# jzhangbs/MVSDF

Measured on AMD Instinct MI355X. Metric: traced rays/sec (fwd+bwd, 10 sphere iters, 4 src views), higher is better.
Workload: dtype f32x3

## Files before the change

### include/mvsdf_hip.h

```cpp
#ifndef MVSDF_HIP_H
#define MVSDF_HIP_H
#include <stddef.h>
#include <stdint.h>

#ifdef __cplusplus
extern "C" {
#endif

#define MVSDF_MAX_LAYERS 12

typedef struct {
    int n_layers;
    int K[MVSDF_MAX_LAYERS];
    int N[MVSDF_MAX_LAYERS];
    const float* wp[MVSDF_MAX_LAYERS];
    const float* bias[MVSDF_MAX_LAYERS];
    const float* w[MVSDF_MAX_LAYERS];
    int skip_layer;
    int multires;
    const void* wp16[MVSDF_MAX_LAYERS];
    int trace_dtype;
    unsigned skip_mask;
    const void* wx3[MVSDF_MAX_LAYERS];
} MvsdfNetDesc;
// ... 32 lines not shown
size_t mvsdf_packed_floats(int N, int K);

int mvsdf_fold_pack(const float* v, const float* g, int N, int K, float* w, float* wp, float* wpT, void* stream);
int mvsdf_fold_pack_net(int n_layers, const float* const* v, const float* const* g, const int* N, const int* K, float* const* w,
                        float* const* wp, float* const* wpT, void* stream);
int mvsdf_fold_backward_net(int n_layers, const float* const* v, const float* const* g, const float* const* dW, const float* const* db,
                            const int* N, const int* K, float* const* dv, float* const* dg, float* const* dbias, int accumulate,
                            void* stream);
int mvsdf_fold_backward(const float* v, const float* g, const float* dW, int N, int K, float* dv, float* dg, void* stream);

size_t mvsdf_packed_bf16_bytes(int N, int K, int nsplit);
int mvsdf_pack_bf16w_net(int n_layers, const float* const* w, const int* N, const int* K, float* const* wp_rounded, void* stream);
int mvsdf_pack_bf16s_net(int n_layers, const float* const* w, const int* N, const int* K, void* const* wp16, void* stream);
int mvsdf_pack_bf16x3_net(int n_layers, const float* const* w, const int* N, const int* K, void* const* wp16, void* stream);
int mvsdf_pack_bf16x3t_net(int n_layers, const float* const* w, const int* N, const int* K, void* const* wx3t, void* stream);

int mvsdf_sdf_col0(const MvsdfNetDesc* net, const float* x, int n, float* y, int mt, void* stream);

int mvsdf_camera_rays(const float* uv, const float* pose, const float* intrinsics, int B, int P, float* ray_dirs, float* cam_loc,
                      void* stream);

int mvsdf_sphere_intersection(const float* cam_loc, const float* ray_dirs, int B, int P, float r, float* t, uint8_t* mask, void* stream);

size_t mvsdf_trace_workspace_bytes(int R);
size_t mvsdf_trace_workspace_bytes_n(int R, int n_steps);
int mvsdf_trace(const MvsdfNetDesc* net, const MvsdfTraceParams* tp, const float* cam_loc, const float* ray_dirs,
                const uint8_t* object_mask, int B, int P, int training, const float* intervals, const float* minsdf_steps,
                float* points, uint8_t* mask, float* dists, unsigned long long* counters, void* workspace,
                size_t workspace_bytes, int mt, int mt_samples, void* stream);
int mvsdf_trace_stage(int stage, const MvsdfNetDesc* net, const MvsdfTraceParams* tp, const float* cam_loc, const float* ray_dirs,
                      const uint8_t* object_mask, int B, int P, int training, const float* intervals, const float* minsdf_steps,
                      float* points, uint8_t* mask, float* dists, unsigned long long* counters, void* workspace,
                      size_t workspace_bytes, int mt, int mt_samples, void* stream);

size_t mvsdf_tracegen_state_bytes(int R);
int mvsdf_tracegen_init(const MvsdfTraceParams* tp, const float* cam_loc, const float* ray_dirs, const uint8_t* object_mask, int B, int P,
                        void* state, uint8_t* req, float* pts, unsigned long long* counters, void* stream);
int mvsdf_tracegen_step(const MvsdfTraceParams* tp, const float* cam_loc, const float* ray_dirs, int B, int P, void* state, const float* vals,
                        uint8_t* req, float* pts, unsigned long long* counters, void* stream);
int mvsdf_tracegen_finish(const MvsdfTraceParams* tp, const float* cam_loc, const float* ray_dirs, int B, int P, int training, const void* state,
                          float* points, uint8_t* mask, float* dists, unsigned long long* counters, void* workspace, size_t workspace_bytes,
                          void* stream);
int mvsdf_tracegen_rows(const MvsdfTraceParams* tp, int kind, const float* cam_loc, const float* ray_dirs, int B, int P, const float* zs, int n_list,
                        void* workspace, float* out_pts, void* stream);
int mvsdf_tracegen_reduce(const MvsdfTraceParams* tp, int kind, const float* cam_loc, const float* ray_dirs, int B, int P, int training,
                          const float* intervals, const float* minsdf_steps, const float* sv, float* points, uint8_t* mask, float* dists,
                          unsigned long long* counters, void* workspace, uint8_t* marks, void* stream);
int mvsdf_tracegen_secant(const MvsdfTraceParams* tp, int op, const float* cam_loc, const float* ray_dirs, int B, int P, int n_sec, const float* vals,
                          float* pts_out, float* points, float* dists, unsigned long long* counters, void* workspace, void* stream);

size_t mvsdf_sdf_ctx_floats(const MvsdfNetDesc* net, int M, int Mg);
int mvsdf_sdf_forward(const MvsdfNetDesc* net, const MvsdfNetDesc* netT, const float* x, int M, int Mg, float* y, float* nrm, float* ctx,
                      void* stream);
size_t mvsdf_sdf_bwd_ws_floats(const MvsdfNetDesc* net, int Mb);
int mvsdf_sdf_backward(const MvsdfNetDesc* net, const MvsdfNetDesc* netT, const float* x, int M, int Mg, int row0, int Mb, const float* dy,
                       const float* dn, const float* ctx, float* dW_cat, float* db_cat, float* dx, float* ws, void* stream);

int mvsdf_sdf_backward_pair(const MvsdfNetDesc* net, const MvsdfNetDesc* netT, int M, int Mg, int MbA, const float* dyA, const float* dnA, float* wsA,
                            int row0X, int MbX, const float* dyX, const float* dnX, float* wsX, float* dx, const float* ctx, void* stream);
int mvsdf_sdf_backward_finish(const MvsdfNetDesc* net, const MvsdfNetDesc* netT, int M, int Mg, int Mb, const float* dy, const float* ctx, float* ws,
                              int row0D, int MbD, const float* fbar, float* dW_cat, float* db_cat, void* stream);

size_t mvsdf_render_ctx_floats(const MvsdfNetDesc* net, int N);
size_t mvsdf_render_bwd_ws_floats(const MvsdfNetDesc* net, int N);
int mvsdf_render_forward(const MvsdfNetDesc* net, const float* points, const float* view, const float* normals, const float* feat,
                         int ldfeat, int N, int multires_view, float* rgb, float* ctx, void* stream);
// ... 278 lines not shown
```

### mvsdf_amd/_lib.py

```python
import ctypes as C
import os

_HERE = os.path.dirname(os.path.abspath(__file__))
SO_PATH = os.environ.get('MVSDF_LIB') or os.path.join(_HERE, 'libmvsdf_hip.so')
MAX_LAYERS = 12
_lib = None


class NetDesc(C.Structure):
    _fields_ = [('n_layers', C.c_int), ('K', C.c_int * MAX_LAYERS), ('N', C.c_int * MAX_LAYERS),
                ('wp', C.c_void_p * MAX_LAYERS), ('bias', C.c_void_p * MAX_LAYERS), ('w', C.c_void_p * MAX_LAYERS),
                ('skip_layer', C.c_int), ('multires', C.c_int), ('wp16', C.c_void_p * MAX_LAYERS), ('trace_dtype', C.c_int), ('skip_mask', C.c_uint), ('wx3', C.c_void_p * MAX_LAYERS)]


class TraceParams(C.Structure):
    _fields_ = [('r', C.c_float), ('thr', C.c_float), ('line_search_step', C.c_float), ('line_step_iters', C.c_int),
                ('st_iters', C.c_int), ('n_steps', C.c_int), ('n_secant', C.c_int), ('dist_clip', C.c_float)]


class MvsdfError(RuntimeError):
    pass


def lib():
    global _lib
    if _lib is None:
        if not os.path.exists(SO_PATH):
            raise MvsdfError('libmvsdf_hip.so not found at %s -- run `python -c "import __graft_entry__ as g; g.build()"` '
                             '(hipcc --offload-arch=gfx950); there is no CPU/PyTorch fallback for the hot path' % SO_PATH)
        import torch
        L = C.CDLL(SO_PATH)
        L.mvsdf_last_error.restype = C.c_char_p
        L.mvsdf_packed_floats.restype = C.c_size_t
        L.mvsdf_packed_floats.argtypes = [C.c_int, C.c_int]
        L.mvsdf_trace_workspace_bytes.restype = C.c_size_t
        L.mvsdf_trace_workspace_bytes.argtypes = [C.c_int]
        L.mvsdf_trace_workspace_bytes_n.restype = C.c_size_t
        L.mvsdf_trace_workspace_bytes_n.argtypes = [C.c_int, C.c_int]
        for fn in ('mvsdf_sdf_ctx_floats', 'mvsdf_sdf_bwd_ws_floats', 'mvsdf_render_ctx_floats', 'mvsdf_render_bwd_ws_floats'):
            getattr(L, fn).restype = C.c_size_t
        L.mvsdf_adam_ws_floats.restype = C.c_size_t
        L.mvsdf_packed_bf16_bytes.restype = C.c_size_t
        L.mvsdf_packed_bf16_bytes.argtypes = [C.c_int, C.c_int, C.c_int]
        L.mvsdf_tracegen_state_bytes.restype = C.c_size_t
        L.mvsdf_adam_step.argtypes = [C.c_void_p] * 4 + [C.c_size_t] + [C.c_float, C.c_double, C.c_double, C.c_float] + [C.c_int, C.c_float, C.c_void_p, C.c_void_p, C.c_void_p]
        L.mvsdf_adam_step_scaled.argtypes = [C.c_void_p] * 4 + [C.c_size_t] + [C.c_float, C.c_double, C.c_double, C.c_float] + [C.c_int, C.c_float, C.c_float, C.c_void_p, C.c_void_p, C.c_void_p]
        L.mvsdf_adam_step_fused.argtypes = [C.c_void_p] * 4 + [C.c_size_t] + [C.c_float, C.c_double, C.c_double, C.c_float] + [C.c_int, C.c_float, C.c_float, C.c_int, C.c_void_p, C.c_void_p, C.c_void_p]
        L.mvsdf_loss_scale.argtypes = [C.c_void_p] + [C.c_float] * 5 + [C.c_void_p, C.c_void_p, C.c_int] * 4 + [C.c_void_p, C.c_void_p]
        i64, vp, f32 = C.c_int64, C.c_void_p, C.c_float
        L.mvsdf_mc_workspace_bytes.restype = C.c_size_t
        L.mvsdf_mc_workspace_bytes.argtypes = [i64] * 3
        L.mvsdf_mc_count.argtypes = [vp, vp, vp, f32, vp, C.c_size_t, vp]
        L.mvsdf_mc_emit.argtypes = [vp, vp, vp, f32, vp, vp, vp, C.c_size_t, vp, vp, vp, i64, i64, vp]
        L.mvsdf_mesh_cc_workspace_bytes.restype = C.c_size_t
        L.mvsdf_mesh_cc_workspace_bytes.argtypes = [i64, i64]
        L.mvsdf_mesh_components.argtypes = [vp, vp, i64, i64, vp, C.c_size_t, vp, vp, vp]
        L.mvsdf_mesh_select.argtypes = [vp, vp, i64, i64, C.c_int32] + [vp] * 5 + [C.c_size_t] + [vp] * 4 + [i64, i64, vp]
        L.mvsdf_smc_workspace_bytes.restype = C.c_size_t
        L.mvsdf_smc_workspace_bytes.argtypes = [i64, i64]
        L.mvsdf_smc_emit_workspace_bytes.restype = C.c_size_t
        L.mvsdf_smc_emit_workspace_bytes.argtypes = [i64, i64, i64]
        L.mvsdf_smc_coarse_points.argtypes = [vp, i64, i64, i64, i64, vp, vp]
        L.mvsdf_smc_seed.argtypes = [vp, i64, i64, f32, f32, vp, C.c_size_t, vp]
        L.mvsdf_smc_brick_points.argtypes = [vp, i64, i64, vp, C.c_size_t, i64, i64, vp, vp]
        L.mvsdf_smc_closure.argtypes = [vp, i64, i64, f32, i64, i64, vp, C.c_size_t, vp]
        L.mvsdf_smc_count.argtypes = [vp, i64, i64, f32, i64, vp, C.c_size_t, vp, C.c_size_t, vp]
        L.mvsdf_smc_emit.argtypes = [vp, i64, i64, f32, vp, vp, i64, vp, C.c_size_t, vp, C.c_size_t, vp, vp, vp, i64, i64, vp]
        L.mvsdf_mesh_cut_workspace_bytes.restype = C.c_size_t
        L.mvsdf_mesh_cut_workspace_bytes.argtypes = [i64, i64]
        L.mvsdf_mesh_cut.argtypes = [vp, vp, i64, i64, C.c_int32, C.c_int32, vp, C.c_size_t, vp, vp]
        L.mvsdf_mesh_trim.argtypes = [vp] * 4 + [i64, i64, vp, C.c_size_t] + [vp] * 4 + [i64, i64, vp]
# ... 33 lines not shown
        L.mvsdf_featext_raw_floats.argtypes = []
        L.mvsdf_featext_pack_bytes.argtypes = []
        L.mvsdf_featext_pack.argtypes = [vp, vp, sz, vp]
        L.mvsdf_featext_workspace_bytes.argtypes = [i64] * 3
        L.mvsdf_featext_forward.argtypes = [vp, vp, i64, i64, i64, vp, sz, vp, vp, vp, C.c_int, C.c_int, vp]
        L.mvsdf_featext_layer_workspace_bytes.argtypes = [C.c_int] * 5
        L.mvsdf_featext_layer.argtypes = [C.c_int, vp, vp, C.c_int, C.c_int, C.c_int, vp, C.c_int, vp, C.c_int, i64, i64, i64, vp, C.c_int, vp, sz, vp, vp]
        for fn in ('mvsdf_stereo_workspace_bytes', 'mvsdf_stereo_volume_offset'):
            getattr(L, fn).restype = sz
            getattr(L, fn).argtypes = [i64] * 4
        L.mvsdf_stereo_normalize.argtypes = [vp, i64, i64, vp, vp, vp]
        L.mvsdf_stereo_patches.argtypes = [vp, i64, i64, i64, i32, vp, vp]
        L.mvsdf_stereo_sweep.argtypes = [vp, i64, i64, i64, i64, i64] + [vp] * 7 + [sz] + [vp] * 5
        L.mvsdf_viewsel_bits_bytes.restype = sz
        L.mvsdf_viewsel_bits_bytes.argtypes = [i64, i64]
        L.mvsdf_viewsel_workspace_bytes.restype = sz
        L.mvsdf_viewsel_workspace_bytes.argtypes = [i64]
        L.mvsdf_viewsel_pack_dense.argtypes = [vp, i64, i64, vp, vp, vp]
        L.mvsdf_viewsel_pack_tracks.argtypes = [vp, vp, i64, i64, i64, vp, vp, vp]
        L.mvsdf_viewsel_scores.argtypes = [vp, vp, vp, i64, i64, f64, f64, f64, vp, sz, vp, vp, vp, vp]
        L.mvsdf_viewsel_depths.argtypes = [vp, vp, vp, i64, i64, i64, i64, vp, vp, vp]
        L.mvsdf_viewsel_weights_host.argtypes = [vp, vp, i64, f64, f64, f64, vp, vp]
        L.mvsdf_batch_args_bytes.restype = sz
        L.mvsdf_batch_args_bytes.argtypes = []
        L.mvsdf_batch_gather.argtypes = [vp, vp]
        for name in EXPORTS:
            getattr(L, name)
        _lib = L
    return _lib


EXPORTS = [
    'mvsdf_version', 'mvsdf_abi_struct_sizes', 'mvsdf_last_error', 'mvsdf_packed_floats', 'mvsdf_fold_pack', 'mvsdf_fold_backward', 'mvsdf_fold_pack_net', 'mvsdf_fold_backward_net', 'mvsdf_packed_bf16_bytes', 'mvsdf_pack_bf16w_net', 'mvsdf_pack_bf16s_net', 'mvsdf_pack_bf16x3_net', 'mvsdf_pack_bf16x3t_net',
    'mvsdf_sdf_col0', 'mvsdf_camera_rays', 'mvsdf_sphere_intersection', 'mvsdf_trace_workspace_bytes', 'mvsdf_trace_workspace_bytes_n', 'mvsdf_trace', 'mvsdf_trace_stage', 'mvsdf_det_math',
    'mvsdf_tracegen_state_bytes', 'mvsdf_tracegen_init', 'mvsdf_tracegen_step', 'mvsdf_tracegen_finish', 'mvsdf_tracegen_rows', 'mvsdf_tracegen_reduce',
    'mvsdf_tracegen_secant',
    'mvsdf_sdf_ctx_floats', 'mvsdf_sdf_forward', 'mvsdf_sdf_bwd_ws_floats', 'mvsdf_sdf_backward', 'mvsdf_sdf_backward_pair', 'mvsdf_sdf_backward_finish',
    'mvsdf_feat_corr', 'mvsdf_depth_carve', 'mvsdf_loss_terms', 'mvsdf_loss_prep', 'mvsdf_loss_scale', 'mvsdf_adam_ws_floats', 'mvsdf_adam_step', 'mvsdf_adam_step_scaled', 'mvsdf_adam_step_fused',
    'mvsdf_partition_rays', 'mvsdf_step_outputs', 'mvsdf_step_backward_inputs', 'mvsdf_step_backward_fbar', 'mvsdf_dsurf_select', 'mvsdf_dsurf_points',
    'mvsdf_render_ctx_floats', 'mvsdf_render_bwd_ws_floats', 'mvsdf_render_forward', 'mvsdf_render_backward',
    'mvsdf_step_create', 'mvsdf_step_destroy', 'mvsdf_step_forward', 'mvsdf_step_wait_counts', 'mvsdf_step_backward', 'mvsdf_step_set_timing', 'mvsdf_step_trace_times', 'mvsdf_step_times',
    'mvsdf_step_seq', 'mvsdf_step_counts_offset', 'mvsdf_step_wait_counts_seq', 'mvsdf_step_done_seq', 'mvsdf_step_can_defer', 'mvsdf_step_saved_offsets',
    'mvsdf_loss_layout', 'mvsdf_loss_forward', 'mvsdf_loss_backward',
    'mvsdf_mc_workspace_bytes', 'mvsdf_mc_count', 'mvsdf_mc_emit', 'mvsdf_mesh_cc_workspace_bytes', 'mvsdf_mesh_components', 'mvsdf_mesh_select',
    'mvsdf_smc_workspace_bytes', 'mvsdf_smc_emit_workspace_bytes', 'mvsdf_smc_coarse_points', 'mvsdf_smc_seed', 'mvsdf_smc_brick_points',
    'mvsdf_smc_closure', 'mvsdf_smc_count', 'mvsdf_smc_emit',
    'mvsdf_mesh_cut_workspace_bytes', 'mvsdf_mesh_cut', 'mvsdf_mesh_trim',
    'mvsdf_chamfer_key', 'mvsdf_chamfer_sample_workspace_bytes', 'mvsdf_chamfer_sample_count', 'mvsdf_chamfer_sample_emit',
    'mvsdf_chamfer_downsample_workspace_bytes', 'mvsdf_chamfer_downsample', 'mvsdf_chamfer_mask_workspace_bytes', 'mvsdf_chamfer_mask',
    'mvsdf_chamfer_nearest_workspace_bytes', 'mvsdf_chamfer_nearest',
    'mvsdf_fusion_workspace_bytes', 'mvsdf_fusion_fuse', 'mvsdf_fusion_emit',
    'mvsdf_cloud_clean_workspace_bytes', 'mvsdf_cloud_compact_workspace_bytes', 'mvsdf_cloud_knn', 'mvsdf_cloud_components', 'mvsdf_cloud_clean',
    'mvsdf_cloud_compact',
    'mvsdf_raster_workspace_bytes', 'mvsdf_raster_draw', 'mvsdf_raster_resolve', 'mvsdf_raster_visibility', 'mvsdf_raster_colors',
    'mvsdf_featext_raw_floats', 'mvsdf_featext_pack_bytes', 'mvsdf_featext_pack', 'mvsdf_featext_workspace_bytes', 'mvsdf_featext_forward',
    'mvsdf_featext_layer_workspace_bytes', 'mvsdf_featext_layer',
    'mvsdf_stereo_workspace_bytes', 'mvsdf_stereo_volume_offset', 'mvsdf_stereo_normalize', 'mvsdf_stereo_patches', 'mvsdf_stereo_sweep',
    'mvsdf_viewsel_bits_bytes', 'mvsdf_viewsel_workspace_bytes', 'mvsdf_viewsel_pack_dense', 'mvsdf_viewsel_pack_tracks', 'mvsdf_viewsel_scores',
    'mvsdf_viewsel_depths', 'mvsdf_viewsel_weights_host',
    'mvsdf_batch_args_bytes', 'mvsdf_batch_gather',
]


def check(rc, what=''):
    if rc != 0:
        raise MvsdfError('%s failed (code %d): %s' % (what or 'mvsdf call', rc, lib().mvsdf_last_error().decode()))

# ... 14 lines not shown
```

### mvsdf_amd/csrc/trace.hip

```cpp
#include <stdlib.h>
#include <type_traits>
#include "tile_engine.h"
#include "tile_engine_bf16.h"
#include "tile_engine_bf16s.h"
#include "trace_params.h"
#include "capi_util.h"

struct RayCommon {
    float c[3], d[3];
};

__device__ __forceinline__ float mv_clamp(float v, float lo, float hi) { return v < lo ? lo : (v > hi ? hi : v); }

__device__ __forceinline__ bool mv_sphere_isect(const float* c, const float* d, float r, float& t0, float& t1) {
    const float dot = fmaf(d[2], c[2], fmaf(d[1], c[1], d[0] * c[0]));
    const float nrm = sqrtf(c[0] * c[0] + c[1] * c[1] + c[2] * c[2]);
    const float under = dot * dot - (nrm * nrm - r * r);
    const bool hit = under > 0.0f;
    float a = 0.0f, b = 0.0f;
    if (hit) {
        const float s = sqrtf(under);
        a = s * -1.0f - dot;
        b = s * 1.0f - dot;
    }
// ... 323 lines not shown
                    }
                }
            }
            for (int o = 32; o > 0; o >>= 1) used += __shfl_xor(used, o);
            if (lane == 0) nrows_total += (unsigned long long)used;
        }
    }

    if (tail.enable) {
        if (tid == 0 && h_units) atomicAdd(&counters[MV_CNT_TAIL_ROWS], (unsigned long long)h_units * (unsigned long long)ROWS);
        if (tail.probe && tid == 0) {
            unsigned* pr = tail.probe + 4 * blockIdx.x;
            pr[0] = n_rounds; pr[1] = h_units; pr[2] = (unsigned)(clk1 - clk0); pr[3] = (unsigned)((long long)wall_clock64() - clk1);
        }
    }
}

struct SampleCtx {
    const float* cam_loc; const float* dirs; int R, P, training, RPW;
    const float* intervals; const float* steps;
    float* o_points; uint8_t* o_mask; float* o_dists;
    const float* w_zmin; const float* w_zmax;
    float* sec_state;
    int* sec_list;
    float* sv;
    int* list_rest; int* src_rest;
    int n_first;
    unsigned long long* counters;
};

struct RowSeg { const int* list; const int* src; int cnt_index, i0, ni, blocks; int unit_rows; };

template <int MT, int NTW, int NW, class NET>
__device__ void mv_eval_rows(const NET& net, const MvTraceParams& tp, const SampleCtx& c, const RowSeg& sg, long long q0, float* smem, int n_list) {
    constexpr int ROWS = 16 * MT;
    const int tid = threadIdx.x;
    const int n_steps = tp.n_steps, ni = sg.ni;
    const long long total = (long long)n_list * ni;
    if (q0 >= total) return;
    const int nr = (int)min((long long)ROWS, total - q0);
    TraceLds lds = mv_carve<NET>(smem, ROWS, net.S, 3 + 6 * net.multires, 0);
    long long svi = 0;
    if (tid < ROWS) {
        float* p = lds.pts + tid * 3;
        if (tid < nr) {
            const long long q = q0 + tid;
            const int it = (int)(q / ni), i = sg.i0 + (int)(q - (long long)it * ni);
            const int e = sg.list[it];
            const int gid = e & 0x0fffffff;
            const bool samp = (e >> 28) & MV_ITEM_SAMPLER;
            const float* cc = c.cam_loc + 3 * (gid / c.P);
            const float* d = c.dirs + 3 * (size_t)gid;
            const float zmin = c.w_zmin[gid], zmax = c.w_zmax[gid];
            const float z = samp ? (zmin + c.intervals[i] * (zmax - zmin))
                                 : (c.steps[i] * (zmax - zmin) + zmin);
            p[0] = cc[0] + z * d[0]; p[1] = cc[1] + z * d[1]; p[2] = cc[2] + z * d[2];
            svi = (long long)(sg.src ? sg.src[it] : it) * n_steps + i;
        } else { p[0] = 0.f; p[1] = 0.f; p[2] = 0.f; }
    }
    __syncthreads();
    mv_eval_dispatch<MT, NTW, NW>(net, (nr + 15) >> 4, lds.act, lds.pe, lds.pts, lds.sdfv, tid);
    if (tid < nr) c.sv[svi] = lds.sdfv[tid];
}

__device__ __forceinline__ int mv_first_where(const float* __restrict__ sv, int n, int lane, int what) {
    for (int base = 0; base < n; base += 64) {
        const int i = base + lane;
        const float v = i < n ? sv[i] : 1.0f;
        const unsigned long long m = __ballot(what == 0 ? (v < 0.f) : (!(v > 0.f) && !(v < 0.f)));
        if (m) return base + __builtin_ctzll(m);
    }
    return -1;
}
// ... 79 lines not shown
                }
            }
        } else {
            if (it == 0 && lead) atomicAdd(&c.counters[MV_CNT_ROWS_MINSDF], (unsigned long long)n_list * (unsigned long long)n_steps);
            const int bi = mv_first_argmin(sv, n_steps, lane);
            if (lead) { dist = c.steps[bi] * (zmax - zmin) + zmin; have_dist = true; }
        }
        if (lead && have_dist) {
            c.o_dists[gid] = dist;
            c.o_points[3 * (size_t)gid + 0] = cc[0] + dist * d[0];
            c.o_points[3 * (size_t)gid + 1] = cc[1] + dist * d[1];
            c.o_points[3 * (size_t)gid + 2] = cc[2] + dist * d[2];
        }
    }
    if (mode == 2) return;
    if (lead) s_cat[w] = cat;
    __syncthreads();
    if (threadIdx.x == 0) {
        unsigned n1 = 0, n2 = 0;
        for (int k = 0; k < MV_RED_WAVES; ++k) { n1 += s_cat[k] == 1; n2 += s_cat[k] == 2; }
        if (n1) s_base[0] = atomicAdd(&c.counters[MV_CNT_N_SAMPLER_REST], (unsigned long long)n1);
        if (n2) s_base[1] = atomicAdd(&c.counters[MV_CNT_N_SECANT], (unsigned long long)n2);
    }
    __syncthreads();
    if (lead && cat) {
        unsigned rank = 0;
        for (int k = 0; k < w; ++k) rank += s_cat[k] == cat;
        const unsigned long long k = s_base[cat - 1] + rank;
        if (cat == 1) { c.list_rest[k] = e; c.src_rest[k] = it; }
        else c.sec_list[k] = gid;
    }
}

template <int MT, int NTW, int NW, class NET>
__device__ void mv_secant_rays(const NET& net, const MvTraceParams& tp, const SampleCtx& c, int n_list, int block, float* smem) {
    constexpr int ROWS = 16 * MT;
    const int tid = threadIdx.x;
    const int r0 = block * ROWS;
    if (r0 >= n_list) return;
    const int n = min(ROWS, n_list - r0);
    TraceLds lds = mv_carve<NET>(smem, ROWS, net.S, 3 + 6 * net.multires, 0);
    const bool mine = tid < n;
    int gid = 0;
    float cc[3] = {0, 0, 0}, d[3] = {0, 0, 0}, z_low = 0, z_high = 0, sdf_low = 0, sdf_high = 1, z_pred = 0;
    if (mine) {
        gid = c.sec_list[r0 + tid];
        const int b = gid / c.P;
        for (int i = 0; i < 3; ++i) { cc[i] = c.cam_loc[3 * b + i]; d[i] = c.dirs[3 * (size_t)gid + i]; }
        z_low = c.sec_state[gid]; z_high = c.sec_state[(size_t)c.R + gid];
        sdf_low = c.sec_state[2 * (size_t)c.R + gid]; sdf_high = c.sec_state[3 * (size_t)c.R + gid];
        z_pred = -sdf_low * (z_high - z_low) / (sdf_high - sdf_low) + z_low;
    }
    for (int it = 0; it < tp.n_secant; ++it) {
        if (tid < ROWS) { float* p = lds.pts + tid * 3; p[0] = cc[0] + z_pred * d[0]; p[1] = cc[1] + z_pred * d[1]; p[2] = cc[2] + z_pred * d[2]; }
        __syncthreads();
        mv_eval_dispatch<MT, NTW, NW>(net, (n + 15) >> 4, lds.act, lds.pe, lds.pts, lds.sdfv, tid);
        if (mine) {
            const float sm = lds.sdfv[tid];
            if (sm > 0.f) { z_low = z_pred; sdf_low = sm; }
            if (sm < 0.f) { z_high = z_pred; sdf_high = sm; }
            z_pred = -sdf_low * (z_high - z_low) / (sdf_high - sdf_low) + z_low;
        }
    }
    if (mine) {
        c.o_dists[gid] = z_pred;
        c.o_points[3 * (size_t)gid + 0] = cc[0] + z_pred * d[0];
        c.o_points[3 * (size_t)gid + 1] = cc[1] + z_pred * d[1];
        c.o_points[3 * (size_t)gid + 2] = cc[2] + z_pred * d[2];
    }
    if (tid == 0) atomicAdd(&c.counters[MV_CNT_ROWS_SECANT], (unsigned long long)n * (unsigned long long)tp.n_secant);
}

template <class NET> struct mv_net_wt { static constexpr int v = 1; };
template <int NS, int WT> struct mv_net_wt<MvNetBs<NS, WT>> { static constexpr int v = WT; };
template <int MT, int NTW, int NW, class NET>
__global__ __launch_bounds__(64 * NW, (mv_net_wt<NET>::v == 3 && NTW == 2 && MT <= 2 && NW == 8) ? 4 : NW / 4) void k_ray_samples(NET net, MvTraceParams tp, SampleCtx c, RowSeg s0, RowSeg s1, int sec_blocks) {
    extern __shared__ __attribute__((aligned(16))) float smem[];
    int b = blockIdx.x;
    if (b < sec_blocks) {
        mv_secant_rays<(MT > 1 ? 1 : MT), NTW, NW, NET>(net, tp, c, (int)c.counters[MV_CNT_N_SECANT], b, smem);
        return;
    }
    b -= sec_blocks;
    const bool first = b < s0.blocks;
    if (!first && b - s0.blocks >= s1.blocks) return;
    const RowSeg sg = first ? s0 : s1;
    long long q0 = (long long)(first ? b : b - s0.blocks) * (16 * MT);
    const int n_list = (int)c.counters[sg.cnt_index];
    if (sg.unit_rows > 0) {
        if (q0 >= (long long)n_list * sg.ni + 16 * MT) return;
        __shared__ long long s_q0;
        if (threadIdx.x == 0) s_q0 = (long long)atomicAdd(&c.counters[MV_CNT_TAIL_NEXT], (unsigned long long)(16 * MT));
        __syncthreads();
        q0 = s_q0;
    }
    mv_eval_rows<MT, NTW, NW, NET>(net, tp, c, sg, q0, smem, n_list);
}
static int mv_tail_mode() {
    static int v = -1;
    if (v < 0) { const char* e = getenv("MVSDF_TAIL"); v = e ? atoi(e) : 1; }
    return v;
}
static unsigned* g_tail_probe = nullptr;
static unsigned* mv_tail_probe() { return g_tail_probe; }
extern "C" void mv_trace_set_tail_probe(unsigned* buf) { g_tail_probe = buf; }
static float* mv_minsdf_sv(float* ws, int R, int n_steps) {
    float* sec_state = ws + 2 * (size_t)R;
    int* w_list = (int*)(sec_state + 4 * (size_t)R);
    float* sv = (float*)(w_list + 3 * (size_t)R);
    int* list_rest = (int*)(sv + (size_t)R * n_steps);
    return (float*)(list_rest + 2 * (size_t)R);
}

static int mv_cu_count() {
    static int n = 0;
    if (n == 0) {
        int dev = 0, v = 0;
        if (hipGetDevice(&dev) != hipSuccess || hipDeviceGetAttribute(&v, hipDeviceAttributeMultiprocessorCount, dev) != hipSuccess || v <= 0) { (void)hipGetLastError(); v = 1; }
        n = v;
    }
    return n;
}
template <class NET>
static bool mv_tail_on(int training, const float* steps, int R, int mt1) {
    constexpr bool is_bf = !std::is_same<NET, MvNet>::value;
    const int grid1 = (R + 8 * mt1 - 1) / (8 * mt1);
    const int need = !is_bf ? 1 : ((mv_net_wt<NET>::v == 3 && R > 2048) ? 1 : 2);
    return training && steps && mv_tail_mode() >= need && grid1 <= mv_cu_count();
}

template <class NET>
static size_t trace_lds_bytes(const NET& net, int MT, int sv_floats, int rpw, bool sphere = false) {
    const int rows = 16 * MT, d0 = 3 + 6 * net.multires;
    size_t f = (size_t)mv_act_rows<NET>(rows, sphere) * net.S + ((rows * d0 + 3) & ~3) + rows * 4 + rows + sv_floats;
    return f * 4 + 16 + (size_t)rpw * (8 * 4 + 4) + 16;
}

template <int MT, int NTW, int NW, class NET>
// ... 33 lines not shown

template <int MT, int NTW, int NW, class NET>
static hipError_t launch_stage2(const NET& net, const MvTraceParams& tp, const float* cam_loc, const float* dirs, int B, int P, int training,
                                const float* intervals, const float* steps, float* points, uint8_t* mask, float* dists, float* ws,
                                unsigned long long* counters, int parts, int mt1, hipStream_t stream) {
    const int R = B * P, ROWS = 16 * MT;
    float* w_zmin = ws;
    float* w_zmax = w_zmin + R;
    float* sec_state = w_zmax + R;
    int* w_list = (int*)(sec_state + 4 * (size_t)R);
    int* w_list_min = w_list + R;
    int* sec_list = w_list_min + R;
    float* sv = (float*)(sec_list + R);
    const size_t lds2 = trace_lds_bytes(net, MT, 0, 0);
    static size_t set2 = 0;
    if (lds2 > set2) {
        hipError_t e = hipFuncSetAttribute((const void*)k_ray_samples<MT, NTW, NW, NET>, hipFuncAttributeMaxDynamicSharedMemorySize, (int)lds2);
        if (e != hipSuccess) return e;
        set2 = lds2;
    }
    static int nf_env = -1;
    if (nf_env < 0) { const char* e = mv_dev_env("MVSDF_NFIRST"); nf_env = e ? atoi(e) : 12; if (nf_env < 2) nf_env = 2; }
    const int n = tp.n_steps, nf = nf_env < n ? nf_env : n;
    SampleCtx c;
    c.cam_loc = cam_loc; c.dirs = dirs; c.R = R; c.P = P; c.training = training; c.RPW = 0; c.intervals = intervals; c.steps = steps;
    c.o_points = points; c.o_mask = mask; c.o_dists = dists; c.w_zmin = w_zmin; c.w_zmax = w_zmax; c.sec_state = sec_state;
    c.sec_list = sec_list; c.sv = sv; c.counters = counters;
    c.list_rest = (int*)(sv + (size_t)R * n); c.src_rest = c.list_rest + R; c.n_first = nf;
    auto blocks_for = [&](int per_item) { return (int)(((long long)R * per_item + ROWS - 1) / ROWS); };
    const int sec_blocks = (R + 15) / 16, red_blocks = (R + MV_RED_WAVES - 1) / MV_RED_WAVES;
    const RowSeg none = {nullptr, nullptr, 0, 0, 1, 0, 0};
    if (parts & 1) {
        const RowSeg first = {w_list, nullptr, (int)MV_CNT_N_SAMPLER, 0, nf, blocks_for(nf), 0};
        hipLaunchKernelGGL((k_ray_samples<MT, NTW, NW, NET>), dim3(first.blocks), dim3(64 * NW), lds2, stream, net, tp, c, first, none, 0);
        hipLaunchKernelGGL(k_reduce_items, dim3(red_blocks), dim3(64 * MV_RED_WAVES), 0, stream, tp, c, w_list, (const int*)nullptr, (int)MV_CNT_N_SAMPLER, 0);
        if (nf < n) {
            const RowSeg rest = {c.list_rest, c.src_rest, (int)MV_CNT_N_SAMPLER_REST, nf, n - nf, blocks_for(n - nf), 0};
            hipLaunchKernelGGL((k_ray_samples<MT, NTW, NW, NET>), dim3(rest.blocks), dim3(64 * NW), lds2, stream, net, tp, c, rest, none, 0);
            hipLaunchKernelGGL(k_reduce_items, dim3(red_blocks), dim3(64 * MV_RED_WAVES), 0, stream, tp, c, c.list_rest, c.src_rest, (int)MV_CNT_N_SAMPLER_REST, 1);
        }
    }
    if (parts & 2) {
        const bool tail = mv_tail_on<NET>(training, steps, R, mt1);
        SampleCtx cm = c;
        if (tail) cm.sv = mv_minsdf_sv(ws, R, n);
        const RowSeg minsdf = {w_list_min, nullptr, (int)MV_CNT_N_MINSDF, 0, n, training ? blocks_for(n) + (tail ? 1 : 0) : 0, tail ? 1 : 0};
        hipLaunchKernelGGL((k_ray_samples<MT, NTW, NW, NET>), dim3(sec_blocks + minsdf.blocks), dim3(64 * NW), lds2, stream, net, tp, cm, minsdf, none,
                           sec_blocks);
        if (training) hipLaunchKernelGGL(k_reduce_items, dim3(red_blocks), dim3(64 * MV_RED_WAVES), 0, stream, tp, cm, w_list_min, (const int*)nullptr, (int)MV_CNT_N_MINSDF, 2);
    }
    if ((parts & 4) && training) {
        SampleCtx c2 = c;
        c2.sv = (float*)(c.src_rest + R);
        const bool tail = mv_tail_on<NET>(training, steps, R, mt1);
        const RowSeg minsdf = {w_list_min, nullptr, (int)MV_CNT_N_MINSDF, 0, n, blocks_for(n) + (tail ? 1 : 0), tail ? 1 : 0};
        hipLaunchKernelGGL((k_ray_samples<MT, NTW, NW, NET>), dim3(minsdf.blocks), dim3(64 * NW), lds2, stream, net, tp, c2, minsdf, none, 0);
        hipLaunchKernelGGL(k_reduce_items, dim3(red_blocks), dim3(64 * MV_RED_WAVES), 0, stream, tp, c2, w_list_min, (const int*)nullptr, (int)MV_CNT_N_MINSDF, 2);
    }
    if (parts & 8)
        hipLaunchKernelGGL((k_ray_samples<MT, NTW, NW, NET>), dim3(sec_blocks), dim3(64 * NW), lds2, stream, net, tp, c, none, none, sec_blocks);
    return hipGetLastError();
}

#ifndef MV_SPHERE_NW16
#define MV_SPHERE_NW16 1
#endif
template <class NET>
hipError_t mv_trace_launch(int stages, const NET& net, const MvTraceParams& tp, int mt1, int mt2, const float* cam_loc, const float* dirs,
                           const uint8_t* om, int B, int P, int training, const float* intervals, const float* steps, float* points,
                           uint8_t* mask, float* dists, float* ws, unsigned long long* counters, hipStream_t stream) {
    int maxnt = 0;
    for (int l = 0; l < net.n_layers - 1; ++l) maxnt = net.L[l].NT > maxnt ? net.L[l].NT : maxnt;
    if (maxnt > 32) return hipErrorInvalidValue;
    constexpr bool is_bf = !std::is_same<NET, MvNet>::value;
    const bool eight = is_bf || maxnt >= 16;
    const bool wide = maxnt > 16;
    hipError_t e = hipSuccess;
    auto eff = [&](int mt) { return wide ? (mt >= 2 ? 2 : 1) : (mt >= 4 ? 4 : (mt >= 2 ? 2 : 1)); };
    const int mt1_eff = eff(mt1), mt2_eff = eff(mt2);
#define MV_S1(MT_, NTW_, NW_) e = launch_stage1<MT_, NTW_, NW_>(net, tp, cam_loc, dirs, om, B, P, training, steps, mt2_eff, points, mask, dists, ws, counters, stream)
#define MV_S2(MT_, NTW_, NW_) e = launch_stage2<MT_, NTW_, NW_>(net, tp, cam_loc, dirs, B, P, training, intervals, steps, points, mask, dists, ws, counters, (stages >> 1) & 15, mt1_eff, stream)
    if (stages & 1) {
        if (eight) {
            if (wide) { if (mt1 >= 2) MV_S1(2, 4, 8); else MV_S1(1, 4, 8); }
            else if (mt1 >= 4) MV_S1(4, 2, 8); else if (mt1 >= 2) MV_S1(2, 2, 8);
            else {
                if constexpr (MV_SPHERE_NW16 != 0 && mv_net_wt<NET>::v == 3) MV_S1(1, 1, 16); else MV_S1(1, 2, 8);
            }
        } else if constexpr (!is_bf) {
            if (wide) { if (mt1 >= 2) MV_S1(2, 8, 4); else MV_S1(1, 8, 4); }
            else if (mt1 >= 4) MV_S1(4, 4, 4); else if (mt1 >= 2) MV_S1(2, 4, 4); else MV_S1(1, 4, 4);
        }
        if (e != hipSuccess) return e;
// ... 276 lines not shown
    if (td == 3)
        e = mv_trace_launch(stages, net2, *tp, mt, rpw, cam_loc, ray_dirs, object_mask, B, P, training, intervals,
                            minsdf_steps ? minsdf_steps : intervals, points, mask, dists, (float*)workspace, counters, s);
    else if (td == 4)
        e = mv_trace_launch(stages, net3, *tp, mt, rpw, cam_loc, ray_dirs, object_mask, B, P, training, intervals,
                            minsdf_steps ? minsdf_steps : intervals, points, mask, dists, (float*)workspace, counters, s);
    else if (td == 5)
        e = mv_trace_launch(stages, net33, *tp, mt, rpw, cam_loc, ray_dirs, object_mask, B, P, training, intervals,
                            minsdf_steps ? minsdf_steps : intervals, points, mask, dists, (float*)workspace, counters, s);
    else
        e = mv_trace_launch(stages, net, *tp, mt, rpw, cam_loc, ray_dirs, object_mask, B, P, training, intervals,
                            minsdf_steps ? minsdf_steps : intervals, points, mask, dists, (float*)workspace, counters, s);
    return mv_check(e, "mvsdf_trace");
}

int mvsdf_trace(const MvsdfNetDesc* desc, const MvsdfTraceParams* tp, const float* cam_loc, const float* ray_dirs,
                const uint8_t* object_mask, int B, int P, int training, const float* intervals, const float* minsdf_steps,
                float* points, uint8_t* mask, float* dists, unsigned long long* counters, void* workspace,
                size_t workspace_bytes, int mt, int rpw, void* stream) {
    return trace_impl(7, desc, tp, cam_loc, ray_dirs, object_mask, B, P, training, intervals, minsdf_steps, points, mask, dists, counters,
                      workspace, workspace_bytes, mt, rpw, stream);
}

int mvsdf_trace_stage(int stage, const MvsdfNetDesc* desc, const MvsdfTraceParams* tp, const float* cam_loc, const float* ray_dirs,
                      const uint8_t* object_mask, int B, int P, int training, const float* intervals, const float* minsdf_steps,
                      float* points, uint8_t* mask, float* dists, unsigned long long* counters, void* workspace,
                      size_t workspace_bytes, int mt, int rpw, void* stream) {
    if (stage < 1 || stage > 6) return mv_fail(-1, "mvsdf_trace_stage: stage must be 1..6");
    static const int bits[7] = {0, 1, 6, 2, 4, 8, 16};
    return trace_impl(bits[stage], desc, tp, cam_loc, ray_dirs, object_mask, B, P, training, intervals, minsdf_steps, points, mask, dists, counters,
                      workspace, workspace_bytes, mt, rpw, stream);
}

int mv_trace_stage1_prezeroed(const MvsdfNetDesc* desc, const MvsdfTraceParams* tp, const float* cam_loc, const float* ray_dirs, const uint8_t* object_mask,
                              int B, int P, int training, const float* intervals, const float* minsdf_steps, float* points, uint8_t* mask, float* dists,
                              unsigned long long* counters, void* workspace, size_t workspace_bytes, int mt, int rpw, void* stream) {
    return trace_impl(1 | 0x100, desc, tp, cam_loc, ray_dirs, object_mask, B, P, training, intervals, minsdf_steps, points, mask, dists, counters,
                      workspace, workspace_bytes, mt, rpw, stream);
}

size_t mvsdf_tracegen_state_bytes(int R) { return (size_t)(R > 0 ? R : 0) * sizeof(GenRay); }

static int tracegen_check(const MvsdfTraceParams* tp, int B, int P) {
    if (!tp || B <= 0 || P <= 0 || (long long)B * P >= (1 << 28)) return mv_fail(-1, "mvsdf_tracegen: bad sizes");
    if (tp->n_steps < 2 || tp->n_steps > 1024 || tp->line_step_iters < 0 || tp->line_step_iters > 30) return mv_fail(-1, "mvsdf_tracegen: tracer parameters out of range");
    return 0;
}

int mvsdf_tracegen_init(const MvsdfTraceParams* tp, const float* cam_loc, const float* ray_dirs, const uint8_t* object_mask, int B, int P,
                        void* state, uint8_t* req, float* pts, unsigned long long* counters, void* stream) {
    int rc = tracegen_check(tp, B, P);
    if (rc) return rc;
    if (!cam_loc || !ray_dirs || !object_mask || !state || !req || !pts || !counters) return mv_fail(-1, "mvsdf_tracegen_init: null argument");
    const int R = B * P;
    hipStream_t s = (hipStream_t)stream;
    hipError_t e = hipMemsetAsync(counters, 0, 16 * sizeof(unsigned long long), s);
    if (e != hipSuccess) return mv_check(e, "mvsdf_tracegen_init: memset");
    hipLaunchKernelGGL(k_gen_init, dim3((R + 255) / 256), dim3(256), 0, s, *tp, cam_loc, ray_dirs, object_mask, R, P, (GenRay*)state, req, pts);
    return mv_check(hipGetLastError(), "mvsdf_tracegen_init");
}

int mvsdf_tracegen_step(const MvsdfTraceParams* tp, const float* cam_loc, const float* ray_dirs, int B, int P, void* state, const float* vals,
                        uint8_t* req, float* pts, unsigned long long* counters, void* stream) {
    int rc = tracegen_check(tp, B, P);
    if (rc) return rc;
    if (!cam_loc || !ray_dirs || !state || !vals || !req || !pts || !counters) return mv_fail(-1, "mvsdf_tracegen_step: null argument");
// ... 78 lines not shown
```

Measured before the change: 1.388 million.

## Balance minsdf row tiles across CUs and let secant use cross-row eval

```diff
diff --git a/include/mvsdf_hip.h b/include/mvsdf_hip.h
--- a/include/mvsdf_hip.h
+++ b/include/mvsdf_hip.h
@@ -88,6 +88,8 @@
                       const uint8_t* object_mask, int B, int P, int training, const float* intervals, const float* minsdf_steps,
                       float* points, uint8_t* mask, float* dists, unsigned long long* counters, void* workspace,
                       size_t workspace_bytes, int mt, int mt_samples, void* stream);
+int mvsdf_trace_row_schedule(long long n_rows, int cus, long long grid_blocks, long long block, int mt_samples, long long* q0, int* nr);
+int mvsdf_trace_set_row_cus(int cus);
 
 size_t mvsdf_tracegen_state_bytes(int R);
 int mvsdf_tracegen_init(const MvsdfTraceParams* tp, const float* cam_loc, const float* ray_dirs, const uint8_t* object_mask, int B, int P,
diff --git a/mvsdf_amd/_lib.py b/mvsdf_amd/_lib.py
--- a/mvsdf_amd/_lib.py
+++ b/mvsdf_amd/_lib.py
@@ -37,6 +37,8 @@
         L.mvsdf_trace_workspace_bytes.argtypes = [C.c_int]
         L.mvsdf_trace_workspace_bytes_n.restype = C.c_size_t
         L.mvsdf_trace_workspace_bytes_n.argtypes = [C.c_int, C.c_int]
+        L.mvsdf_trace_row_schedule.argtypes = [C.c_longlong, C.c_int, C.c_longlong, C.c_longlong, C.c_int, C.POINTER(C.c_longlong), C.POINTER(C.c_int)]
+        L.mvsdf_trace_set_row_cus.argtypes = [C.c_int]
         for fn in ('mvsdf_sdf_ctx_floats', 'mvsdf_sdf_bwd_ws_floats', 'mvsdf_render_ctx_floats', 'mvsdf_render_bwd_ws_floats'):
             getattr(L, fn).restype = C.c_size_t
         L.mvsdf_adam_ws_floats.restype = C.c_size_t
@@ -136,7 +138,7 @@
 
 EXPORTS = [
     'mvsdf_version', 'mvsdf_abi_struct_sizes', 'mvsdf_last_error', 'mvsdf_packed_floats', 'mvsdf_fold_pack', 'mvsdf_fold_backward', 'mvsdf_fold_pack_net', 'mvsdf_fold_backward_net', 'mvsdf_packed_bf16_bytes', 'mvsdf_pack_bf16w_net', 'mvsdf_pack_bf16s_net', 'mvsdf_pack_bf16x3_net', 'mvsdf_pack_bf16x3t_net',
-    'mvsdf_sdf_col0', 'mvsdf_camera_rays', 'mvsdf_sphere_intersection', 'mvsdf_trace_workspace_bytes', 'mvsdf_trace_workspace_bytes_n', 'mvsdf_trace', 'mvsdf_trace_stage', 'mvsdf_det_math',
+    'mvsdf_sdf_col0', 'mvsdf_camera_rays', 'mvsdf_sphere_intersection', 'mvsdf_trace_workspace_bytes', 'mvsdf_trace_workspace_bytes_n', 'mvsdf_trace', 'mvsdf_trace_stage', 'mvsdf_trace_row_schedule', 'mvsdf_trace_set_row_cus', 'mvsdf_det_math',
     'mvsdf_tracegen_state_bytes', 'mvsdf_tracegen_init', 'mvsdf_tracegen_step', 'mvsdf_tracegen_finish', 'mvsdf_tracegen_rows', 'mvsdf_tracegen_reduce',
     'mvsdf_tracegen_secant',
     'mvsdf_sdf_ctx_floats', 'mvsdf_sdf_forward', 'mvsdf_sdf_bwd_ws_floats', 'mvsdf_sdf_backward', 'mvsdf_sdf_backward_pair', 'mvsdf_sdf_backward_finish',
diff --git a/mvsdf_amd/csrc/trace.hip b/mvsdf_amd/csrc/trace.hip
--- a/mvsdf_amd/csrc/trace.hip
+++ b/mvsdf_amd/csrc/trace.hip
@@ -379,13 +379,13 @@
 struct RowSeg { const int* list; const int* src; int cnt_index, i0, ni, blocks; int unit_rows; };
 
 template <int MT, int NTW, int NW, class NET>
-__device__ void mv_eval_rows(const NET& net, const MvTraceParams& tp, const SampleCtx& c, const RowSeg& sg, long long q0, float* smem, int n_list) {
+__device__ void mv_eval_rows(const NET& net, const MvTraceParams& tp, const SampleCtx& c, const RowSeg& sg, long long q0, int lim, float* smem, int n_list) {
     constexpr int ROWS = 16 * MT;
     const int tid = threadIdx.x;
     const int n_steps = tp.n_steps, ni = sg.ni;
     const long long total = (long long)n_list * ni;
     if (q0 >= total) return;
-    const int nr = (int)min((long long)ROWS, total - q0);
+    const int nr = (int)min((long long)lim, total - q0);
     TraceLds lds = mv_carve<NET>(smem, ROWS, net.S, 3 + 6 * net.multires, 0);
     long long svi = 0;
     if (tid < ROWS) {
@@ -531,7 +531,7 @@
     }
 }
 
-template <int MT, int NTW, int NW, class NET>
+template <int MT, int NTW, int NW, class NET, bool XR = false>
 __device__ void mv_secant_rays(const NET& net, const MvTraceParams& tp, const SampleCtx& c, int n_list, int block, float* smem) {
     constexpr int ROWS = 16 * MT;
     const int tid = threadIdx.x;
@@ -553,7 +553,7 @@
     for (int it = 0; it < tp.n_secant; ++it) {
         if (tid < ROWS) { float* p = lds.pts + tid * 3; p[0] = cc[0] + z_pred * d[0]; p[1] = cc[1] + z_pred * d[1]; p[2] = cc[2] + z_pred * d[2]; }
         __syncthreads();
-        mv_eval_dispatch<MT, NTW, NW>(net, (n + 15) >> 4, lds.act, lds.pe, lds.pts, lds.sdfv, tid);
+        mv_eval_dispatch<MT, NTW, NW, NET, (XR && MT == 1)>(net, (n + 15) >> 4, lds.act, lds.pe, lds.pts, lds.sdfv, tid);
         if (mine) {
             const float sm = lds.sdfv[tid];
             if (sm > 0.f) { z_low = z_pred; sdf_low = sm; }
@@ -572,12 +572,31 @@
 
 template <class NET> struct mv_net_wt { static constexpr int v = 1; };
 template <int NS, int WT> struct mv_net_wt<MvNetBs<NS, WT>> { static constexpr int v = WT; };
+
+#ifndef MV_ROWS_BALANCED
+#define MV_ROWS_BALANCED 1
+#endif
+#ifndef MV_SECANT_CARRY
+#define MV_SECANT_CARRY 1
+#endif
+__host__ __device__ inline void mv_row_schedule(long long n_rows, long long C, long long grid, long long b, int rows, long long* q0, int* nr) {
+    const long long nfull = (n_rows / (rows * C)) * C;
+    if (b < nfull) { *q0 = b * rows; *nr = rows; return; }
+    const long long base = nfull * rows, rem = n_rows - base;
+    *q0 = n_rows; *nr = 0;
+    if (rem <= 0) return;
+    long long u = 16 * ((rem + 16 * C - 1) / (16 * C));
+    while (u < rows && nfull + (rem + u - 1) / u > grid) u += 16;
+    const long long s = base + (b - nfull) * u;
+    if (s < n_rows) { *q0 = s; *nr = (int)(n_rows - s < u ? n_rows - s : u); }
+}
+
 template <int MT, int NTW, int NW, class NET>
-__global__ __launch_bounds__(64 * NW, (mv_net_wt<NET>::v == 3 && NTW == 2 && MT <= 2 && NW == 8) ? 4 : NW / 4) void k_ray_samples(NET net, MvTraceParams tp, SampleCtx c, RowSeg s0, RowSeg s1, int sec_blocks) {
+__global__ __launch_bounds__(64 * NW, (mv_net_wt<NET>::v == 3 && NTW == 2 && MT <= 2 && NW == 8) ? 4 : NW / 4) void k_ray_samples(NET net, MvTraceParams tp, SampleCtx c, RowSeg s0, RowSeg s1, int sec_blocks, int row_cus) {
     extern __shared__ __attribute__((aligned(16))) float smem[];
     int b = blockIdx.x;
     if (b < sec_blocks) {
-        mv_secant_rays<(MT > 1 ? 1 : MT), NTW, NW, NET>(net, tp, c, (int)c.counters[MV_CNT_N_SECANT], b, smem);
+        mv_secant_rays<(MT > 1 ? 1 : MT), NTW, NW, NET, (MV_SECANT_CARRY != 0 && MT >= 4 && NW == 8)>(net, tp, c, (int)c.counters[MV_CNT_N_SECANT], b, smem);
         return;
     }
     b -= sec_blocks;
@@ -593,7 +612,15 @@
         __syncthreads();
         q0 = s_q0;
     }
-    mv_eval_rows<MT, NTW, NW, NET>(net, tp, c, sg, q0, smem, n_list);
+    int lim = 16 * MT;
+    constexpr bool HELD128 = mv_net_wt<NET>::v == 3 && NTW == 2 && MT <= 2 && NW == 8;
+    if (MV_ROWS_BALANCED != 0 && !HELD128 && row_cus != 0 && first && sg.unit_rows == 0) {
+        const long long sec_active = ((long long)c.counters[MV_CNT_N_SECANT] + 15) >> 4;
+        const long long C = row_cus < 0 ? -(long long)row_cus : (row_cus - sec_active > 1 ? row_cus - sec_active : 1);
+        mv_row_schedule((long long)n_list * sg.ni, C, s0.blocks, b, 16 * MT, &q0, &lim);
+        if (lim == 0) return;
+    }
+    mv_eval_rows<MT, NTW, NW, NET>(net, tp, c, sg, q0, lim, smem, n_list);
 }
 static int mv_tail_mode() {
     static int v = -1;
@@ -603,6 +630,7 @@
 static unsigned* g_tail_probe = nullptr;
 static unsigned* mv_tail_probe() { return g_tail_probe; }
 extern "C" void mv_trace_set_tail_probe(unsigned* buf) { g_tail_probe = buf; }
+static int g_row_cus = 0;
 static float* mv_minsdf_sv(float* ws, int R, int n_steps) {
     float* sec_state = ws + 2 * (size_t)R;
     int* w_list = (int*)(sec_state + 4 * (size_t)R);
@@ -702,11 +730,11 @@
     const RowSeg none = {nullptr, nullptr, 0, 0, 1, 0, 0};
     if (parts & 1) {
         const RowSeg first = {w_list, nullptr, (int)MV_CNT_N_SAMPLER, 0, nf, blocks_for(nf), 0};
-        hipLaunchKernelGGL((k_ray_samples<MT, NTW, NW, NET>), dim3(first.blocks), dim3(64 * NW), lds2, stream, net, tp, c, first, none, 0);
+        hipLaunchKernelGGL((k_ray_samples<MT, NTW, NW, NET>), dim3(first.blocks), dim3(64 * NW), lds2, stream, net, tp, c, first, none, 0, 0);
         hipLaunchKernelGGL(k_reduce_items, dim3(red_blocks), dim3(64 * MV_RED_WAVES), 0, stream, tp, c, w_list, (const int*)nullptr, (int)MV_CNT_N_SAMPLER, 0);
         if (nf < n) {
             const RowSeg rest = {c.list_rest, c.src_rest, (int)MV_CNT_N_SAMPLER_REST, nf, n - nf, blocks_for(n - nf), 0};
-            hipLaunchKernelGGL((k_ray_samples<MT, NTW, NW, NET>), dim3(rest.blocks), dim3(64 * NW), lds2, stream, net, tp, c, rest, none, 0);
+            hipLaunchKernelGGL((k_ray_samples<MT, NTW, NW, NET>), dim3(rest.blocks), dim3(64 * NW), lds2, stream, net, tp, c, rest, none, 0, 0);
             hipLaunchKernelGGL(k_reduce_items, dim3(red_blocks), dim3(64 * MV_RED_WAVES), 0, stream, tp, c, c.list_rest, c.src_rest, (int)MV_CNT_N_SAMPLER_REST, 1);
         }
     }
@@ -716,7 +744,7 @@
         if (tail) cm.sv = mv_minsdf_sv(ws, R, n);
         const RowSeg minsdf = {w_list_min, nullptr, (int)MV_CNT_N_MINSDF, 0, n, training ? blocks_for(n) + (tail ? 1 : 0) : 0, tail ? 1 : 0};
         hipLaunchKernelGGL((k_ray_samples<MT, NTW, NW, NET>), dim3(sec_blocks + minsdf.blocks), dim3(64 * NW), lds2, stream, net, tp, cm, minsdf, none,
-                           sec_blocks);
+                           sec_blocks, (!training || tail) ? 0 : (g_row_cus > 0 ? -g_row_cus : mv_cu_count()));
         if (training) hipLaunchKernelGGL(k_reduce_items, dim3(red_blocks), dim3(64 * MV_RED_WAVES), 0, stream, tp, cm, w_list_min, (const int*)nullptr, (int)MV_CNT_N_MINSDF, 2);
     }
     if ((parts & 4) && training) {
@@ -724,11 +752,11 @@
         c2.sv = (float*)(c.src_rest + R);
         const bool tail = mv_tail_on<NET>(training, steps, R, mt1);
         const RowSeg minsdf = {w_list_min, nullptr, (int)MV_CNT_N_MINSDF, 0, n, blocks_for(n) + (tail ? 1 : 0), tail ? 1 : 0};
-        hipLaunchKernelGGL((k_ray_samples<MT, NTW, NW, NET>), dim3(minsdf.blocks), dim3(64 * NW), lds2, stream, net, tp, c2, minsdf, none, 0);
+        hipLaunchKernelGGL((k_ray_samples<MT, NTW, NW, NET>), dim3(minsdf.blocks), dim3(64 * NW), lds2, stream, net, tp, c2, minsdf, none, 0, 0);
         hipLaunchKernelGGL(k_reduce_items, dim3(red_blocks), dim3(64 * MV_RED_WAVES), 0, stream, tp, c2, w_list_min, (const int*)nullptr, (int)MV_CNT_N_MINSDF, 2);
     }
     if (parts & 8)
-        hipLaunchKernelGGL((k_ray_samples<MT, NTW, NW, NET>), dim3(sec_blocks), dim3(64 * NW), lds2, stream, net, tp, c, none, none, sec_blocks);
+        hipLaunchKernelGGL((k_ray_samples<MT, NTW, NW, NET>), dim3(sec_blocks), dim3(64 * NW), lds2, stream, net, tp, c, none, none, sec_blocks, 0);
     return hipGetLastError();
 }
 
@@ -1071,6 +1099,19 @@
                       workspace, workspace_bytes, mt, rpw, stream);
 }
 
+int mvsdf_trace_row_schedule(long long n_rows, int cus, long long grid_blocks, long long block, int mt_samples, long long* q0, int* nr) {
+    if (n_rows < 0 || cus < 1 || grid_blocks < 0 || block < 0 || mt_samples < 1 || mt_samples > 4 || !q0 || !nr)
+        return mv_fail(1, "mvsdf_trace_row_schedule: bad argument");
+    if (block >= grid_blocks) { *q0 = n_rows; *nr = 0; return 0; }
+    mv_row_schedule(n_rows, cus, grid_blocks, block, 16 * mt_samples, q0, nr);
+    return 0;
+}
+int mvsdf_trace_set_row_cus(int cus) {
+    if (cus < 0) return mv_fail(1, "mvsdf_trace_set_row_cus: cus must be >= 0 (0: the device's count)");
+    g_row_cus = cus;
+    return 0;
+}
+
 int mv_trace_stage1_prezeroed(const MvsdfNetDesc* desc, const MvsdfTraceParams* tp, const float* cam_loc, const float* ray_dirs, const uint8_t* object_mask,
                               int B, int P, int training, const float* intervals, const float* minsdf_steps, float* points, uint8_t* mask, float* dists,
                               unsigned long long* counters, void* workspace, size_t workspace_bytes, int mt, int rpw, void* stream) {
```

New measurement: 1.396 million, median of 5. About the same (+0.6%).
